# LeoIV/polyaxon

Measured on AMD Instinct MI355X. Metric: HPO trials/hour (whole node) + wall-clock-to-target, ResNet-50 Hyperband sweep, higher is better.
Workload: dtype bf16

## Files before the change

polyaxon_amd/csrc/bn_kernels.hip:

```cpp
#include <hip/hip_runtime.h>

#include "handoff.h"
#include <stdint.h>
#include <type_traits>

#define PLX_API extern "C" __attribute__((visibility("default")))

namespace {

constexpr int kBlock = 256;

struct alignas(16) bf16x8 {
  uint16_t v[8];
};

__device__ __forceinline__ float bf2f(uint16_t b) { return __uint_as_float(((uint32_t)b) << 16); }

__device__ __forceinline__ uint16_t f2bf(float f) {
  return __builtin_bit_cast(uint16_t, (__bf16)f);
}

__device__ __forceinline__ void load8(const bf16x8* p, float* f) {
  const bf16x8 v = *p;
#pragma unroll
// ... 81 lines not shown
                                                               float* __restrict__ out, int S) {
  constexpr int G = NT / 64;
  __shared__ float sh[NT];
  const int c = blockIdx.x * 64 + (threadIdx.x & 63);
  const int lane = threadIdx.x >> 6;
  const int s = blockIdx.y, which = blockIdx.z;
  const int b0 = s * kRowsPerSplit;
  const int b1 = b0 + kRowsPerSplit < nblk ? b0 + kRowsPerSplit : nblk;
  sh[threadIdx.x] = c < C ? l1_rows<NT>(part + (int64_t)which * nblk * C, b0, b1, C, c, lane) : 0.f;
  __syncthreads();
  if (lane == 0 && c < C) {
    float r = 0.f;
#pragma unroll
    for (int g = 0; g < G; ++g) r += sh[threadIdx.x + 64 * g];
    out[((int64_t)which * S + s) * C + c] = r;
  }
}

template <int NT = 256, bool ATOMIC = false>
__device__ __forceinline__ bool fin_sum2(const float* __restrict__ pa, const float* __restrict__ pb, int nblk, int C,
                                         double& A, double& B) {
  constexpr int G = NT / 64;
  __shared__ double sh[2][G][64];
  const int lc = threadIdx.x & 63, sp = threadIdx.x >> 6;
  const int c = blockIdx.x * 64 + lc;
  double a0 = 0.0, b0 = 0.0;
  if (c < C) {
    for (int b = sp; b < nblk; b += 8 * G) {
      float x[8], y[8];
#pragma unroll
      for (int u = 0; u < 8; ++u) {
        const int r = b + u * G;
        if (ATOMIC) {
          x[u] = r < nblk ? __hip_atomic_load(pa + (int64_t)r * C + c, __ATOMIC_RELAXED, __HIP_MEMORY_SCOPE_AGENT) : 0.f;
          y[u] = r < nblk ? __hip_atomic_load(pb + (int64_t)r * C + c, __ATOMIC_RELAXED, __HIP_MEMORY_SCOPE_AGENT) : 0.f;
        } else {
          x[u] = r < nblk ? pa[(int64_t)r * C + c] : 0.f;
          y[u] = r < nblk ? pb[(int64_t)r * C + c] : 0.f;
        }
      }
#pragma unroll
      for (int u = 0; u < 8; ++u) { a0 += x[u]; b0 += y[u]; }
    }
  }
  sh[0][sp][lc] = a0;
  sh[1][sp][lc] = b0;
  __syncthreads();
  if (sp != 0 || c >= C) return false;
  double sa = 0.0, sb = 0.0;
#pragma unroll
  for (int g = 0; g < G; ++g) { sa += sh[0][g][lc]; sb += sh[1][g][lc]; }
  A = sa;
  B = sb;
  return true;
}

struct FwdFin {
  const uint16_t* x_row0;
  int C;
  int64_t M;
  const float* gamma;
  const float* beta;
  float eps, momentum;
  float* running_mean;
  float* running_var;
  float* save_mean;
  float* save_invstd;
  float* scale;
  float* bias;
};

struct BwdFin {
  int C;
  int64_t M;
  const float* gamma;
  const float* mean;
  const float* invstd;
  float* dgamma;
  float* dbeta;
  float* coef;
  int accumulate;
};

template <int NT, bool ATOMIC = false>
__device__ __forceinline__ void fwd_finalize(const float* psum, const float* psq, int nblk, const FwdFin& f) {
  double S, Q;
  if (!fin_sum2<NT, ATOMIC>(psum, psq, nblk, f.C, S, Q)) return;
  const int c = blockIdx.x * 64 + (threadIdx.x & 63);
  const double m = S / (double)f.M;
  double var = Q / (double)f.M - m * m;
  if (var < 0.0) var = 0.0;
  const float mean = (f.x_row0 != nullptr ? bf2f(f.x_row0[c]) : 0.f) + (float)m;
  const float invstd = rsqrtf((float)var + f.eps);
  const float g = f.gamma[c];
  f.save_mean[c] = mean;
  f.save_invstd[c] = invstd;
  f.scale[c] = g * invstd;
  f.bias[c] = f.beta[c] - mean * g * invstd;
  if (f.running_mean != nullptr) {
    const float unbiased = f.M > 1 ? (float)(var * (double)f.M / (double)(f.M - 1)) : (float)var;
    f.running_mean[c] = (1.f - f.momentum) * f.running_mean[c] + f.momentum * mean;
    f.running_var[c] = (1.f - f.momentum) * f.running_var[c] + f.momentum * unbiased;
  }
}

template <int NT, bool ATOMIC = false>
__device__ __forceinline__ void bwd_finalize(const float* pdz, const float* pdzx, int nblk, const BwdFin& f) {
  double A, B;
  if (!fin_sum2<NT, ATOMIC>(pdz, pdzx, nblk, f.C, A, B)) return;
  const int C = f.C;
  const int c = blockIdx.x * 64 + (threadIdx.x & 63);
  const float db = (float)A, dg = (float)B;
  f.dbeta[c] = f.accumulate ? f.dbeta[c] + db : db;
  f.dgamma[c] = f.accumulate ? f.dgamma[c] + dg : dg;
  const float is = f.invstd[c], k1 = f.gamma[c] * is;
  const float k2 = db / (float)f.M, k3 = dg / (float)f.M;
  f.coef[c] = k1;
  f.coef[C + c] = -k1 * k3 * is;
  f.coef[2 * C + c] = -k1 * k2 + k1 * k3 * is * f.mean[c];
}

template <int NT>
__device__ __forceinline__ bool reduce_l2_last(const float* __restrict__ part, int nblk, int C, float* l2, int S,
                                               unsigned* cnt) {
  constexpr int G = NT / 64;
  __shared__ float sh[2][NT];
  __shared__ int s_last;
  const int c = blockIdx.x * 64 + (threadIdx.x & 63);
  const int lane = threadIdx.x >> 6;
  const int s = blockIdx.y;
  const int b0 = s * kRowsPerSplit;
  int b1 = b0 + kRowsPerSplit;
  if (b1 > nblk) b1 = nblk;
  float a0 = 0.f, a1 = 0.f;
  if (c < C) {
    a0 = l1_rows<NT>(part, b0, b1, C, c, lane);
    a1 = l1_rows<NT>(part + (int64_t)nblk * C, b0, b1, C, c, lane);
  }
  sh[0][threadIdx.x] = a0;
  sh[1][threadIdx.x] = a1;
  __syncthreads();
  if (lane == 0 && c < C) {
    const int t = threadIdx.x;
    float r0 = 0.f, r1 = 0.f;
#pragma unroll
    for (int g = 0; g < G; ++g) { r0 += sh[0][t + 64 * g]; r1 += sh[1][t + 64 * g]; }
    __hip_atomic_store(l2 + (int64_t)s * C + c, r0, __ATOMIC_RELAXED, __HIP_MEMORY_SCOPE_AGENT);
    __hip_atomic_store(l2 + ((int64_t)S + s) * C + c, r1, __ATOMIC_RELAXED, __HIP_MEMORY_SCOPE_AGENT);
  }
  asm volatile("s_waitcnt vmcnt(0)" ::: "memory");
  __syncthreads();
  if (threadIdx.x == 0) {
    plx_handoff_release();
    const unsigned old = __hip_atomic_fetch_add(cnt + blockIdx.x, 1u, __ATOMIC_RELAXED, __HIP_MEMORY_SCOPE_AGENT);
    const int last = old == (unsigned)(S - 1);
    if (last) plx_handoff_acquire();
    if (last) __hip_atomic_store(cnt + blockIdx.x, 0u, __ATOMIC_RELAXED, __HIP_MEMORY_SCOPE_AGENT);
    s_last = last;
  }
  __syncthreads();
  return s_last != 0;
}

constexpr int kFinNT = 1024;
template <int NT>
__global__ __launch_bounds__(NT) void bn_fwd_reduce_finalize_kernel(const float* __restrict__ part, int nblk, float* l2,
                                                                    int S, unsigned* cnt, FwdFin f) {
  if (!reduce_l2_last<NT>(part, nblk, f.C, l2, S, cnt)) return;
  fwd_finalize<NT, true>(l2, l2 + (int64_t)S * f.C, S, f);
}

template <int NT>
__global__ __launch_bounds__(NT) void bn_bwd_reduce_finalize_kernel(const float* __restrict__ part, int nblk, float* l2,
                                                                    int S, unsigned* cnt, BwdFin f) {
  if (!reduce_l2_last<NT>(part, nblk, f.C, l2, S, cnt)) return;
  bwd_finalize<NT, true>(l2, l2 + (int64_t)S * f.C, S, f);
}

template <int NT>
__global__ __launch_bounds__(NT) void bn_fwd_finalize_kernel(const float* __restrict__ psum, const float* __restrict__ psq, int nblk,
                                       const uint16_t* __restrict__ x_row0, int C, int64_t M,
                                       const float* __restrict__ gamma, const float* __restrict__ beta, float eps,
                                       float momentum, float* __restrict__ running_mean,
                                       float* __restrict__ running_var, float* __restrict__ save_mean,
                                       float* __restrict__ save_invstd, float* __restrict__ scale,
                                       float* __restrict__ bias) {
  double S, Q;
  if (!fin_sum2<NT>(psum, psq, nblk, C, S, Q)) return;
  const int c = blockIdx.x * 64 + (threadIdx.x & 63);
  const double m = S / (double)M;
  double var = Q / (double)M - m * m;
  if (var < 0.0) var = 0.0;
  const float mean = (x_row0 != nullptr ? bf2f(x_row0[c]) : 0.f) + (float)m;
  const float invstd = rsqrtf((float)var + eps);
  const float g = gamma[c];
  save_mean[c] = mean;
  save_invstd[c] = invstd;
  scale[c] = g * invstd;
  bias[c] = beta[c] - mean * g * invstd;
  if (running_mean != nullptr) {
    const float unbiased = M > 1 ? (float)(var * (double)M / (double)(M - 1)) : (float)var;
    running_mean[c] = (1.f - momentum) * running_mean[c] + momentum * mean;
    running_var[c] = (1.f - momentum) * running_var[c] + momentum * unbiased;
  }
}

template <bool RES, bool RELU>
__global__ __launch_bounds__(kBlock) void bn_apply_kernel(const bf16x8* __restrict__ x, const bf16x8* __restrict__ res,
                                                          bf16x8* __restrict__ y, const float* __restrict__ scale,
                                                          const float* __restrict__ bias, int64_t n_vec, int G,
                                                          uint8_t* __restrict__ mask, const float* __restrict__ rsb) {
  const int64_t stride = (int64_t)gridDim.x * blockDim.x;
  int64_t i = (int64_t)blockIdx.x * blockDim.x + threadIdx.x;
  if (i >= n_vec) return;
  const int cg = (int)(i % G);
  float a[8], b[8], ra[8], rb[8];
#pragma unroll
  for (int k = 0; k < 8; ++k) {
    a[k] = scale[cg * 8 + k];
    b[k] = bias[cg * 8 + k];
    ra[k] = 1.f;
    rb[k] = 0.f;
  }
  if (RES && rsb != nullptr) {
#pragma unroll
    for (int k = 0; k < 8; ++k) {
      ra[k] = rsb[cg * 8 + k];
      rb[k] = rsb[G * 8 + cg * 8 + k];
    }
  }
  for (; i < n_vec; i += stride) {
    const bf16x8 xv = x[i];
    bf16x8 rv;
    if constexpr (RES) rv = res[i];
    float v[8];
#pragma unroll
    for (int k = 0; k < 8; ++k) v[k] = fmaf(bf2f(xv.v[k]), a[k], b[k]);
    if constexpr (RES) {
#pragma unroll
      for (int k = 0; k < 8; ++k) v[k] += fmaf(bf2f(rv.v[k]), ra[k], rb[k]);
    }
    if constexpr (RELU) {
#pragma unroll
      for (int k = 0; k < 8; ++k) v[k] = fmaxf(v[k], 0.f);
    }
    store8(y + i, v);
    if (RELU && mask != nullptr) {
      uint32_t bits = 0;
#pragma unroll
      for (int k = 0; k < 8; ++k) bits |= (uint32_t)(v[k] > 0.f) << k;
      mask[i] = (uint8_t)bits;
    }
  }
}

template <bool RELU>
__global__ __launch_bounds__(kBlock) void bn_bwd_reduce_kernel(const bf16x8* __restrict__ x, const uint8_t* __restrict__ mask,
                                                               const bf16x8* __restrict__ dy, int64_t M, int G, int Gb,
                                                               int64_t rows_per_block, const float* __restrict__ mean,
// ... 138 lines not shown
  for (int k = 0; k < 8; ++k) {
    red[threadIdx.x * 16 + k] = ra[k];
    red[threadIdx.x * 16 + 8 + k] = rc[k];
  }
  __syncthreads();
  if ((int)threadIdx.x < G) {
    for (int j = 1; j < kBlock / G; ++j) {
      const float* o = red + (j * G + threadIdx.x) * 16;
#pragma unroll
      for (int k = 0; k < 8; ++k) {
        ra[k] += o[k];
        rc[k] += o[8 + k];
      }
    }
    float* pa = rb.part + (int64_t)blockIdx.x * C + cg * 8;
    float* pc = rb.part + ((int64_t)gridDim.x + blockIdx.x) * C + cg * 8;
#pragma unroll
    for (int k = 0; k < 8; ++k) {
      pa[k] = ra[k];
      pc[k] = rc[k];
    }
  }
  }
}

struct Plan {
  int G, Gb, gy, nblk, S;
  int64_t rows_per_block;
};

inline bool plan_for(int64_t M, int C, Plan* p) {
  if (M < 1 || C <= 0 || (C & 7)) return false;
  const int G = C / 8;
  if (G & (G - 1)) return false;
  p->G = G;
  p->Gb = G < kBlock ? G : kBlock;
  p->gy = G / p->Gb;
  const int R = kBlock / p->Gb;
  const int64_t cap = (2048 + p->gy - 1) / p->gy;
  int64_t want = (M + 16 * R - 1) / (16 * R);
  if (want > cap) want = cap;
  if (want < 1) want = 1;
  int64_t rpb = (M + want - 1) / want;
  rpb = (rpb + R - 1) / R * R;
  p->rows_per_block = rpb;
  p->nblk = (int)((M + rpb - 1) / rpb);
  p->S = (p->nblk + kRowsPerSplit - 1) / kRowsPerSplit;
  return true;
}

inline int apply_grid(int64_t n_vec, int G) {
  int64_t g = (n_vec + kBlock - 1) / kBlock;
  if (g > 4096) g = 4096;
  if (g < 1) g = 1;
  const int64_t mult = G > kBlock ? G / kBlock : 1;
  g = (g + mult - 1) / mult * mult;
  return (int)g;
}

inline void launch_dx(hipStream_t stream, int64_t n_vec, int G, const void* x, const uint8_t* mask, const void* dy,
                      void* dx, void* dres, const float* coef, int relu, const ResBn& rb) {
  const dim3 grid(apply_grid(n_vec, G));
  auto pick = [&](auto d) {
    constexpr bool DRES = decltype(d)::value;
    return rb.part == nullptr
               ? (relu ? bn_bwd_dx_kernel<false, true, false, DRES> : bn_bwd_dx_kernel<false, false, false, DRES>)
           : rb.mask != nullptr
               ? (relu ? bn_bwd_dx_kernel<true, true, true, DRES> : bn_bwd_dx_kernel<true, false, true, DRES>)
               : (relu ? bn_bwd_dx_kernel<true, true, false, DRES> : bn_bwd_dx_kernel<true, false, false, DRES>);
  };
  auto k = dres != nullptr ? pick(std::true_type{}) : pick(std::false_type{});
  hipLaunchKernelGGL(k, grid, dim3(kBlock), 0, stream, (const bf16x8*)x, mask, (const bf16x8*)dy, (bf16x8*)dx,
                     (bf16x8*)dres, coef, n_vec, G, relu, rb);
}

inline void launch_apply(hipStream_t stream, int64_t n_vec, int G, const void* x, const void* res, void* y,
                         const float* scale, const float* bias, int relu, uint8_t* mask, const float* rsb) {
  auto k = res != nullptr ? (relu ? bn_apply_kernel<true, true> : bn_apply_kernel<true, false>)
                          : (relu ? bn_apply_kernel<false, true> : bn_apply_kernel<false, false>);
  hipLaunchKernelGGL(k, dim3(apply_grid(n_vec, G)), dim3(kBlock), 0, stream, (const bf16x8*)x, (const bf16x8*)res,
                     (bf16x8*)y, scale, bias, n_vec, G, mask, rsb);
}

inline void reduce_finalize_fwd(hipStream_t stream, const float* part, int nblk, float* l2, unsigned* cnt,
                                const FwdFin& f) {
  const int C = f.C, S = (nblk + kRowsPerSplit - 1) / kRowsPerSplit;
  if (cnt != nullptr) {
    hipLaunchKernelGGL(bn_fwd_reduce_finalize_kernel<kFinNT>, dim3((C + 63) / 64, S), dim3(kFinNT), 0, stream, part, nblk, l2, S,
                       cnt, f);
    return;
  }
  hipLaunchKernelGGL(bn_partial_reduce_kernel<kFinNT>,
                     dim3((C + 63) / 64, S, 2), dim3(kFinNT), 0, stream, part, nblk, C, l2, S);
  hipLaunchKernelGGL(bn_fwd_finalize_kernel<kFinNT>, dim3((C + 63) / 64),
                     dim3(kFinNT), 0, stream, l2, l2 + (int64_t)S * C, S,
                     f.x_row0, C, f.M, f.gamma, f.beta, f.eps, f.momentum, f.running_mean, f.running_var, f.save_mean,
                     f.save_invstd, f.scale, f.bias);
}

inline void reduce_finalize_bwd(hipStream_t stream, const float* part, int nblk, float* l2, unsigned* cnt,
                                const BwdFin& f) {
  const int C = f.C, S = (nblk + kRowsPerSplit - 1) / kRowsPerSplit;
  if (cnt != nullptr) {
    hipLaunchKernelGGL(bn_bwd_reduce_finalize_kernel<kFinNT>, dim3((C + 63) / 64, S), dim3(kFinNT), 0, stream, part, nblk, l2, S,
                       cnt, f);
    return;
  }
  hipLaunchKernelGGL(bn_partial_reduce_kernel<kFinNT>,
                     dim3((C + 63) / 64, S, 2), dim3(kFinNT), 0, stream, part, nblk, C, l2, S);
  hipLaunchKernelGGL(bn_bwd_finalize_kernel<kFinNT>, dim3((C + 63) / 64),
                     dim3(kFinNT), 0, stream, l2, l2 + (int64_t)S * C, S, C,
                     f.M, f.gamma, f.mean, f.invstd, f.dgamma, f.dbeta, f.coef, f.accumulate);
}

struct alignas(8) u8x8 {
  uint8_t v[8];
};

__global__ __launch_bounds__(256) void stem_apply_pool_kernel(const bf16x8* __restrict__ x,
                                                              const float* __restrict__ sb, bf16x8* __restrict__ y,
                                                              u8x8* __restrict__ idx, int N, int H, int W, int G,
                                                              int OH, int OW) {
  const unsigned j = blockIdx.x * 256u + threadIdx.x;
  if (j >= (unsigned)(OW * G)) return;
  const unsigned g = j % (unsigned)G, ow = j / (unsigned)G;
  const int C = G * 8;
  float a[8], b[8];
#pragma unroll
  for (int k = 0; k < 8; ++k) {
    a[k] = sb[g * 8 + k];
    b[k] = sb[C + g * 8 + k];
  }
  for (int row = blockIdx.y; row < N * OH; row += gridDim.y) {
    const int n = row / OH, oh = row - n * OH;
    float best[8];
    uint8_t arg[8];
#pragma unroll
    for (int k = 0; k < 8; ++k) {
      best[k] = -INFINITY;
      arg[k] = 255;
    }
    uint4 q[9];
    bool ok[9];
#pragma unroll
    for (int kh = 0; kh < 3; ++kh) {
      const int ih = oh * 2 - 1 + kh;
      const int ihc = ih < 0 ? 0 : (ih >= H ? H - 1 : ih);
#pragma unroll
      for (int kw = 0; kw < 3; ++kw) {
        const int iw = (int)ow * 2 - 1 + kw;
        const int iwc = iw < 0 ? 0 : (iw >= W ? W - 1 : iw);
        ok[kh * 3 + kw] = ih >= 0 && ih < H && iw >= 0 && iw < W;
        q[kh * 3 + kw] = *(const uint4*)(x + ((size_t)(n * H + ihc) * W + iwc) * G + g);
      }
    }
#pragma unroll
    for (int t9 = 0; t9 < 9; ++t9) {
      const uint32_t qw[4] = {q[t9].x, q[t9].y, q[t9].z, q[t9].w};
#pragma unroll
      for (int k = 0; k < 8; ++k) {
        const float xk = __uint_as_float((k & 1) ? (qw[k >> 1] & 0xffff0000u) : (qw[k >> 1] << 16));
        const float f = (float)(__bf16)fmaxf(fmaf(xk, a[k], b[k]), 0.f);
        if (ok[t9] && (f > best[k] || arg[k] == 255)) {
          best[k] = f;
          arg[k] = (uint8_t)t9;
        }
      }
    }
    bf16x8 o;
    u8x8 m;
#pragma unroll
    for (int k = 0; k < 8; ++k) {
      o.v[k] = f2bf(best[k]);
      m.v[k] = arg[k];
    }
    const size_t t = (size_t)row * OW * G + j;
    y[t] = o;
    idx[t] = m;
  }
}

__device__ __forceinline__ int stem_cover(int i, int O, int* o, int* k) {
  int n = 0;
  if (i & 1) {
    if ((i + 1) >> 1 < O) { o[n] = (i + 1) >> 1; k[n++] = 0; }
// ... 292 lines not shown
    for (int h = 0; h < 2; ++h) {
      float cst[NA][4];
#pragma unroll
      for (int arr = 0; arr < NA; ++arr) {
        const float4 v = thin_lds[(arr * 2 + h) * G + g];
        cst[arr][0] = v.x, cst[arr][1] = v.y, cst[arr][2] = v.z, cst[arr][3] = v.w;
      }
      thin_pin4(amw[0][h], amw[1][h], amw[2][h], amw[3][h]);
#pragma unroll
      for (int kp = 0; kp < 2; ++kp) {
        const int w = h * 2 + kp;
        thin_pin4(dw[0][w], dw[1][w], dw[2][w], dw[3][w]);
        thin_pin4(xw[0][w], xw[1][w], xw[2][w], xw[3][w]);
#pragma unroll
        for (int k2 = 0; k2 < 2; ++k2) {
          const int kk = kp * 2 + k2, k = h * 4 + kk;
#pragma unroll
          for (int e = 0; e < 4; ++e) {
            const int di = e >> 1, dj = e & 1;
            float acc = 0.f;
#pragma unroll
            for (int p = 0; p < 2; ++p)
#pragma unroll
              for (int q = 0; q < 2; ++q) {
                const int kh = di + 1 - 2 * p, kw = dj + 1 - 2 * q;
                if (kh < 0 || kw < 0) continue;
                const int w4 = p * 2 + q;
                const uint32_t ab = amw[w4][h] >> (8 * kk) & 0xffu;
                const float dv = __uint_as_float(k2 ? (dw[w4][w] & 0xffff0000u) : (dw[w4][w] << 16));
                acc += ab == (uint32_t)(kh * 3 + kw) ? dv : 0.f;
              }
            const float xf = __uint_as_float(k2 ? (xw[e][w] & 0xffff0000u) : (xw[e][w] << 16));
            const float dz = (pv[e] && fmaf(xf, cst[0][kk], cst[1][kk]) > 0.f) ? (float)(__bf16)acc : 0.f;
            if constexpr (DX) {
              const uint32_t ob = f2bf(fmaf(cst[2][kk], dz, fmaf(cst[3][kk], xf, cst[NA - 1][kk])));
              ow4[e][w] = k2 ? (ow4[e][w] | (ob << 16)) : ob;
            } else {
              s1[k] += dz;
              s2[k] = fmaf(dz, (xf - cst[2][kk]) * cst[3][kk], s2[k]);
            }
          }
        }
        if constexpr (DX) thin_pin4(ow4[0][w], ow4[1][w], ow4[2][w], ow4[3][w]);
        thin_sched_fence();
      }
    }
    if constexpr (DX) {
#pragma unroll
      for (int e = 0; e < 4; ++e)
        if (pv[e])
          *(uint4*)(dx + ((size_t)(n * H + 2 * qa + (e >> 1)) * W + 2 * qb + (e & 1)) * G + g) =
              make_uint4(ow4[e][0], ow4[e][1], ow4[e][2], ow4[e][3]);
    }
  }
  if constexpr (!DX) {
    __shared__ float red[256 * 17];
#pragma unroll
    for (int k = 0; k < 8; ++k) {
      red[threadIdx.x * 17 + k] = s1[k];
      red[threadIdx.x * 17 + 8 + k] = s2[k];
    }
    __syncthreads();
    const int nb = gridDim.x * gridDim.y, blk = blockIdx.y * gridDim.x + blockIdx.x;
    for (int e = threadIdx.x; e < G * 16; e += 256) {
      const int gg = e % G, v = e / G;
      float sum = 0.f;
      for (int r = gg; r < 256; r += G) sum += red[r * 17 + v];
      const int c = gg * 8 + (v & 7);
      part[((int64_t)(v < 8 ? 0 : nb) + blk) * C + c] = sum;
    }
  }
}

constexpr int g_stem_bwd_cap = 4096;

inline dim3 stem_bwd_grid(int N, int H, int W, int G, bool dx) {
  const int rows = N * ((H + 1) / 2), cap = dx ? 65535 : g_stem_bwd_cap;
  return dim3((((W + 1) / 2) * G + 255) / 256, rows < cap ? rows : cap);
}

}

PLX_API void plx_bn_set_thin(int on) { g_bn_thin = on != 0; }

PLX_API int64_t plx_bn_workspace(int64_t M, int C) {
  Plan p;
  if (!plan_for(M, C, &p)) return -1;
  return 2 * (int64_t)(p.nblk + p.S) * C;
}

PLX_API int64_t plx_bn_l2_workspace(int nblk, int C) {
  return 2 * (int64_t)((nblk + kRowsPerSplit - 1) / kRowsPerSplit) * C;
}

PLX_API int plx_bn_dx_blocks(int64_t M, int C) {
  Plan p;
  if (!plan_for(M, C, &p)) return -1;
  return apply_grid(M * p.G, p.G);
}

struct BnForwardArgs {
  const void *x, *res;
  void* y;
  int64_t M;
  int C, relu;
  const float *gamma, *beta;
  float eps, momentum;
  float *running_mean, *running_var;
  float *save_mean, *save_invstd, *scale_bias , *workspace;
  const float* ext_part;
  int ext_nblk;
  uint8_t* mask;
  const float* res_sb;
  unsigned* counters;
};

struct BnBackwardArgs {
  const void* x;
  const uint8_t* mask;
  const void* dy;
  void* dx;
  void* dres;
  int64_t M;
  int C, relu;
  const float *gamma, *save_mean, *save_invstd;
  float *dgamma, *dbeta, *coef , *workspace;
  const float* ext_part;
  int ext_nblk, accumulate;
  ResBn resbn;
  unsigned* counters;
  int no_dres;
};

PLX_API int plx_bn_args_size(int backward) {
  return (int)(backward ? sizeof(BnBackwardArgs) : sizeof(BnForwardArgs));
}

PLX_API int plx_bn_forward(const BnForwardArgs* a, hipStream_t stream) {
  Plan p;
  const int C = a->C;
  if (!plan_for(a->M, C, &p) || (a->ext_part != nullptr && a->ext_nblk < 1)) return 1;
  const bool own = a->ext_part == nullptr;
  const int nblk = own ? p.nblk : a->ext_nblk;
  float* l2 = own ? a->workspace + 2 * (int64_t)nblk * C : a->workspace;
  if (own)
    hipLaunchKernelGGL(bn_stats_kernel, dim3(p.nblk, p.gy), dim3(kBlock), 0, stream, (const bf16x8*)a->x, a->M, p.G,
                       p.Gb, p.rows_per_block, a->workspace, a->workspace + (int64_t)nblk * C);
  reduce_finalize_fwd(stream, own ? a->workspace : a->ext_part, nblk, l2, a->counters,
                      FwdFin{own ? (const uint16_t*)a->x : nullptr, C, a->M, a->gamma, a->beta, a->eps, a->momentum, a->running_mean,
                             a->running_var, a->save_mean, a->save_invstd, a->scale_bias, a->scale_bias + C});
  if (a->y != nullptr)
    launch_apply(stream, a->M * p.G, p.G, a->x, a->res, a->y, a->scale_bias, a->scale_bias + C, a->relu,
                 a->relu ? a->mask : nullptr, a->res_sb);
  return (int)hipGetLastError();
}

PLX_API int plx_bn_backward(const BnBackwardArgs* a, hipStream_t stream) {
  Plan p;
  const int C = a->C, relu = a->relu;
  const ResBn& rb = a->resbn;
  const bool has_rb = rb.x != nullptr || rb.mask != nullptr || rb.mean != nullptr || rb.invstd != nullptr ||
                      rb.part != nullptr;
  if (!plan_for(a->M, C, &p) || (a->ext_part != nullptr && a->ext_nblk < 1)) return 1;
  if (relu && a->mask == nullptr && (a->ext_part == nullptr || a->dx != nullptr)) return 1;
  if (has_rb && (rb.part == nullptr || rb.x == nullptr || rb.mean == nullptr || rb.invstd == nullptr)) return 1;
  if (has_rb && (a->dres == nullptr) != (a->no_dres != 0)) return 1;
// ... 105 lines not shown
```

polyaxon_amd/ops/_native.py:

```python
from __future__ import annotations

import ctypes
import hashlib
import os
import shutil
import subprocess
import threading
from pathlib import Path
from typing import Dict, Iterable, List, Optional

PKG_DIR = Path(__file__).resolve().parent.parent
CSRC = PKG_DIR / "csrc"
OUT = PKG_DIR / "_native"
ARCH = os.environ.get("PLX_OFFLOAD_ARCH", "gfx950")
ROCM = Path(os.environ.get("ROCM_PATH", "/opt/rocm"))

LIBRARIES: Dict[str, dict] = {
    "plx_train": {"sources": ["train_kernels.hip"], "kind": "hip", "link": []},
    "plx_polytune": {"sources": ["polytune_kernels.hip"], "kind": "hip", "link": []},
    "plx_bn": {"sources": ["bn_kernels.hip"], "kind": "hip", "link": []},
    "plx_procmon": {"sources": ["procmon.cpp"], "kind": "cpp", "link": ["-lpthread"]},
    "plx_gp": {"sources": ["gp_kernels.hip", "gp_chol.hip"], "kind": "hip", "link": []},
    "plx_rms": {"sources": ["rmsnorm.hip"], "kind": "hip", "link": []},
    "plx_conv": {"sources": ["conv_gemm.hip"], "kind": "hip", "link": []},
# ... 65 lines not shown
    return out


def _stale(name: str) -> bool:
    spec = LIBRARIES[name]
    stamp = lib_path(name).with_suffix(".so.sha")
    if not stamp.exists():
        return False
    try:
        digest = _digest([CSRC / s for s in spec["sources"]], _flags(spec["kind"]) + spec["link"])
    except OSError:
        return False
    return stamp.read_text().strip() != digest


def build_all(force: bool = False, verbose: bool = False) -> List[Path]:
    return [build(n, force=force, verbose=verbose) for n in LIBRARIES]


def available(name: str) -> bool:
    return lib_path(name).exists()


_SIZES: Dict[tuple, int] = {}


_COUNTERS: Dict[tuple, object] = {}


def capturing() -> bool:
    import torch

    return torch.cuda.is_available() and torch.cuda.is_current_stream_capturing()


def cached(cache: dict, key, make, ok=None):
    v = cache.get(key)
    if v is not None and (ok is None or ok(v)):
        return v
    v = make()
    if not capturing():
        cache[key] = v
    return v


def counters(device, key: str, n: int = 4096):
    import torch

    return cached(_COUNTERS, (str(device), key), lambda: torch.zeros(n, dtype=torch.int32, device=device))


def current_stream() -> int:
    import torch

    return torch._C._cuda_getCurrentRawStream(torch._C._cuda_getDevice())


def size(libname: str, fn: str, *args: int) -> int:
    key = (fn,) + args
    v = _SIZES.get(key)
    if v is None:
        v = _SIZES[key] = int(getattr(lib(libname), fn)(*args))
    return v


def lib(name: str) -> ctypes.CDLL:
    with _lock:
        if name in _loaded:
            return _loaded[name]
        path = lib_path(name)
        if not path.exists() or os.environ.get("PLX_NATIVE_REBUILD") == "1" or _stale(name):
            build(name, force=os.environ.get("PLX_NATIVE_REBUILD") == "1")
        handle = ctypes.CDLL(str(path), mode=ctypes.RTLD_GLOBAL)
        _declare(name, handle)
        if name == "plx_bn":
            for backward, image in enumerate((BnForwardArgs, BnBackwardArgs)):
                if handle.plx_bn_args_size(backward) != ctypes.sizeof(image):
                    raise RuntimeError(f"{image.__name__} layout mismatch: HIP {handle.plx_bn_args_size(backward)} vs "
                                       f"ctypes {ctypes.sizeof(image)}")
        if name == "plx_conv" and os.environ.get("PLX_WGRAD_ATOMIC"):
            handle.plx_set_tn_atomic(int(os.environ["PLX_WGRAD_ATOMIC"]))
        if name == "plx_bn" and os.environ.get("PLX_BN_THIN"):
            handle.plx_bn_set_thin(int(os.environ["PLX_BN_THIN"]))
        if name == "plx_gemm" and os.environ.get("PLX_GEMM_WAVES"):
            handle.plx_gemm256_set_waves(int(os.environ["PLX_GEMM_WAVES"]))
        _loaded[name] = handle
        return handle


_P = ctypes.c_void_p
_I = ctypes.c_int
_L = ctypes.c_int64
_U64 = ctypes.c_uint64
_F = ctypes.c_float
_D = ctypes.c_double

SIGNATURES: Dict[str, Dict[str, list]] = {
    "plx_train": {
        "plx_sgd_flat": [_P, _P, _P, _L, _L, _P, _P, _P],
        "plx_adamw_flat": [_P, _P, _P, _P, _L, _L, _P, _P, _P],
        "plx_adamw_mixed": [_P, _P, _P, _P, _P, _L, _I, _P, _P, _P],
        "plx_sgd_flat_clip": [_P, _P, _P, _L, _L, _P, _P, _P, _P],
        "plx_adamw_flat_clip": [_P, _P, _P, _P, _L, _L, _P, _P, _P, _P],
        "plx_adamw_mixed_clip": [_P, _P, _P, _P, _P, _L, _I, _P, _P, _P, _P],
        "plx_gradnorm_blocks": [_L],
        "plx_gradnorm_partials": [_P, _I, _L, _P, _P],
        "plx_gradnorm_finalize": [_P, _I, _P, _P, _P],
        "plx_lr_schedule": [_P, _P, _P, _P],
        "plx_cast_lp": [_P, _P, _L, _P],
        "plx_init_flat": [_P, _P, _P, _P, _I, _P, _P, _U64, _P],
        "plx_zero_flat": [_P, _L, _P],
        "plx_record_metric": [_P, _I, _P, _P, _I, _P],
        "plx_commit_metric": [_P, _P, _I, _I, _P, _I, _P],
        "plx_synth_images": [_P, _P, _I, _I, _I, _P, _I, _I, _F, _U64, _P, _P],
        "plx_set_adamw_grid_cap": [_I],
        "plx_set_adamw_wide": [_I],
    },
    "plx_bn": {
        "plx_bn_set_thin": [_I],
        "plx_bn_workspace": [_L, _I],
        "plx_bn_args_size": [_I],
        "plx_bn_forward": [_P, _P],
        "plx_bn_apply": [_P, _P, _P, _L, _I, _P, _I, _P],
        "plx_bn_apply_res_relu": [_P, _P, _P, _L, _I, _P, _P, _P, _P],
        "plx_bn_l2_workspace": [_I, _I],
        "plx_bn_backward": [_P, _P],
        "plx_bn_dx_blocks": [_L, _I],
        "plx_stem_bn_pool_forward": [_P, _P, _P, _I, _I, _I, _I, _P, _P, _F, _F, _P, _P, _P, _P, _P, _P, _P, _I, _P,
                                     _P],
        "plx_stem_bn_pool_bwd_workspace": [_I, _I, _I, _I],
        "plx_stem_bn_pool_backward": [_P, _P, _P, _P, _I, _I, _I, _I, _P, _P, _P, _P, _P, _P, _P, _P, _I, _P, _P],
    },
    "plx_procmon": {
        "plx_pm_create": [],
        "plx_pm_destroy": [_P],
        "plx_pm_spawn": [_P, _P, _P, ctypes.c_char_p, ctypes.c_char_p, ctypes.POINTER(_I)],
        "plx_pm_wait": [_P, _I, ctypes.POINTER(_I), ctypes.POINTER(_I)],
        "plx_pm_wake": [_P],
        "plx_pm_signal": [_P, _I, _I, _I],
        "plx_pm_count": [_P],
    },
    "plx_gp": {
        "plx_gp_kmat": [_P, _P, _I, _I, _I, _P, _I, _I, _F, _F, _F, _I, _F, _P, _P, _D, _I, _P],
        "plx_gp_chol": [_P, _I, _I, _P, _P],
        "plx_gp_kmat_batch_f64": [_P, _I, _I, _P, _I, _P, _I, _L, _I, _D, _D, _D, _P, _P, _D, _I, _P],
        "plx_gp_matern_table": [_D, _D, _D, _I, _P, _P, _P],
        "plx_gp_chol_aug_f64": [_P, _I, _I, _I, _L, _I, _P, _P, _P],
        "plx_gp_chol_scratch_doubles": [],
        "plx_gp_lml_f64": [_P, _I, _I, _L, _I, _P, _P, _P],
        "plx_gp_acq_rows": [_P, _I, _I, _P, _F, _I, _F, _F, _F, _P, _P, _P, _P],
        "plx_gp_predict_acq": [_P, _I, _P, _I, _I, _P, _I, _P, _I, _F, _F, _F, _F, _I, _F, _F, _F, _P, _P, _P, _P,
                               _P, _P, _P, _D, _I, _P],
        "plx_gp_ascent": [_P, _P, _I, _P, _P, _P, _I, _I, _P, _P, _I, _F, _F, _F, _F, _I, _F, _F, _F, _I, _P, _P, _D, _I,
                          _P],
    },
    "plx_conv": {
        "plx_gemm_nt": [_P, _P, _P, _I, _I, _I, _I, _I, _I, _P, _P, _I, _P, _P, _P],
        "plx_gemm_nt_bndx": [_P, _P, _P, _P, _P, _P, _P, _I, _I, _I, _I, _I, _P, _I, _P, _P, _P],
        "plx_gemm_nt_bndx_wgrad": [_P, _P, _P, _P, _P, _P, _P, _I, _I, _I, _I, _I, _P, _I, _P, _P, _P, _P, _I, _I, _P],
        "plx_gemm_nt_bnapply": [_P, _P, _P, _P, _P, _P, _P, _P, _I, _I, _I, _I, _I, _P, _P],
        "plx_gemm_nt_rows_per_block": [_I],
        "plx_gemm_nt_plan": [_I, _I, _I, _I],
        "plx_gemm_tn_workspace": [_I, _I, _I, _I],
        "plx_set_tn_v2": [_I, _I],
        "plx_set_tn2_stem": [_I],
        "plx_set_tn2_c64": [_I],
        "plx_set_tn_atomic": [_I],
        "plx_get_tn_atomic": [],
        "plx_tn_plan_slices": [_I, _I, _I, _I, _I],
        "plx_gemm_tn": [_P, _P, _P, _P, _I, _I, _I, _I, _I, _I, _I, _I, _P],
        "plx_weight_prep": [_P, _P, _P, _I, _I, _P],
        "plx_weight_prepk": [_P, _L, _L, _L, _L, _P, _P, _I, _I, _I, _P],
        "plx_weight_prep_all": [_P, _P, _P, _P, _I, _I, _P],
        "plx_stem_pack_input": [_P, _P, _I, _I, _I, _P],
        "plx_stem_pack_weight": [_P, _L, _L, _L, _L, _P, _I, _P],
        "plx_stem_conv_fwd": [_P, _P, _P, _I, _I, _I, _P, _P],
        "plx_stem_conv_wgrad_workspace": [_I, _I, _I, _I],
        "plx_stem_conv_wgrad": [_P, _P, _P, _L, _L, _L, _L, _P, _I, _I, _I, _I, _I, _P],
        "plx_conv_fwd": [_P, _P, _P, _I, _I, _I, _I, _I, _I, _I, _P, _P],
        "plx_conv_dgrad": [_P, _P, _P, _I, _I, _I, _I, _I, _I, _I, _P, _P, _P],
        "plx_conv_dgrad_blocks": [_I, _I, _I, _I, _I, _I, _I],
        "plx_conv_wgrad_workspace": [_I, _I, _I, _I, _I, _I, _I, _I],
        "plx_conv_wgrad": [_P, _P, _P, _P, _I, _I, _I, _I, _I, _I, _I, _I, _I, _P],
    },
    "plx_lm": {
        "plx_qkv_rope_fwd": [_P, _P, _P, _P, _P, _P, _L, _I, _I, _I, _I, _I, _P],
        "plx_qkv_rope_bwd": [_P, _P, _P, _P, _P, _P, _L, _I, _I, _I, _I, _I, _P],
        "plx_swiglu_fwd": [_P, _P, _L, _I, _P],
        "plx_swiglu_bwd": [_P, _P, _P, _L, _I, _P],
        "plx_xent_fwd": [_P, _P, _P, _P, _I, _I, _I, _P],
        "plx_xent_bwd": [_P, _P, _P, _P, _P, _I, _I, _I, _P],
        "plx_xent_cls_fwd": [_P, _P, _P, _P, _I, _I, _P],
        "plx_xent_cls_bwd": [_P, _P, _P, _P, _P, _I, _I, _F, _P],
        "plx_xent_hp_fwd": [_P, _P, _P, _P, _P, _P, _I, _I, _I, _I, _P],
        "plx_xent_hp_bwd": [_P, _P, _P, _P, _P, _P, _I, _I, _I, _I, _P],
        "plx_xent_cls_hp_fwd": [_P, _P, _P, _P, _P, _P, _I, _I, _I, _P],
        "plx_xent_cls_hp_bwd": [_P, _P, _P, _P, _P, _P, _I, _I, _I, _F, _P],
        "plx_colsum_splits": [_L, _I],
        "plx_colsum": [_P, _L, _I, _P, _P, _P, _I, _P],
        "plx_gelu_bwd_colsum": [_P, _P, _P, _L, _I, _P, _P, _P, _I, _P],
    },
    "plx_gemm": {
# ... 113 lines not shown
```

Measured before the change: 13290.

## Add single-kernel BN stat finalize replacing ticket-based split reduction

Adds a single-launch finalize path for BN forward and backward. When the partial-row count is small, one 1024-thread block per 64 channels reduces all partial sums through shared memory, which removes the multi-block atomic ticket handoff and the L2 scratch round-trip. Per-channel parameters (gamma, beta, running stats, and so on) are now prefetched with bounds-checked buffer loads issued alongside the partial loads, so their latency overlaps the reduction. The ticket path also switches to buffer loads. The trade-off is fewer blocks in flight on the reduction, which lowers parallelism for large channel counts, plus more code paths to keep correct.

Measured after the change: 13460, median of 6. 1.01x the previous value.

```diff
diff --git a/polyaxon_amd/csrc/bn_kernels.hip b/polyaxon_amd/csrc/bn_kernels.hip
--- a/polyaxon_amd/csrc/bn_kernels.hip
+++ b/polyaxon_amd/csrc/bn_kernels.hip
@@ -187,42 +187,104 @@
   int accumulate;
 };
 
-template <int NT, bool ATOMIC = false>
-__device__ __forceinline__ void fwd_finalize(const float* psum, const float* psq, int nblk, const FwdFin& f) {
-  double S, Q;
-  if (!fin_sum2<NT, ATOMIC>(psum, psq, nblk, f.C, S, Q)) return;
-  const int c = blockIdx.x * 64 + (threadIdx.x & 63);
+struct FwdPar {
+  float gamma, beta, rmean, rvar, x0;
+};
+
+struct BwdPar {
+  float gamma, mean, invstd, dgamma, dbeta;
+};
+
+__device__ __forceinline__ __amdgpu_buffer_rsrc_t buf_rsrc(const void* p, int bytes) {
+  return __builtin_amdgcn_make_buffer_rsrc(const_cast<void*>(p), 0, bytes, 0x00020000);
+}
+
+__device__ __forceinline__ float par_load(const float* p, int C, int c, bool on) {
+  const int bytes = p != nullptr ? C * (int)sizeof(float) : 0;
+  return __uint_as_float(__builtin_amdgcn_raw_buffer_load_b32(buf_rsrc(p, bytes), on ? c * (int)sizeof(float) : bytes, 0, 0));
+}
+
+__device__ __forceinline__ FwdPar fwd_params(const FwdFin& f, int c, bool on) {
+  FwdPar p;
+  p.gamma = par_load(f.gamma, f.C, c, on);
+  p.beta = par_load(f.beta, f.C, c, on);
+  p.rmean = par_load(f.running_mean, f.C, c, on);
+  p.rvar = par_load(f.running_mean != nullptr ? f.running_var : nullptr, f.C, c, on);
+  const int xbytes = f.x_row0 != nullptr ? 2 * f.C : 0;
+  p.x0 = bf2f((uint16_t)__builtin_amdgcn_raw_buffer_load_b16(buf_rsrc(f.x_row0, xbytes), on ? 2 * c : xbytes, 0, 0));
+  return p;
+}
+
+__device__ __forceinline__ BwdPar bwd_params(const BwdFin& f, int c, bool on) {
+  BwdPar p;
+  p.gamma = par_load(f.gamma, f.C, c, on);
+  p.mean = par_load(f.mean, f.C, c, on);
+  p.invstd = par_load(f.invstd, f.C, c, on);
+  p.dgamma = par_load(f.dgamma, f.C, c, on);
+  p.dbeta = par_load(f.dbeta, f.C, c, on);
+  return p;
+}
+
+__device__ __forceinline__ void fwd_finish(const FwdFin& f, int c, double S, double Q, const FwdPar& p) {
   const double m = S / (double)f.M;
   double var = Q / (double)f.M - m * m;
   if (var < 0.0) var = 0.0;
-  const float mean = (f.x_row0 != nullptr ? bf2f(f.x_row0[c]) : 0.f) + (float)m;
+  const float mean = p.x0 + (float)m;
   const float invstd = rsqrtf((float)var + f.eps);
-  const float g = f.gamma[c];
+  const float g = p.gamma;
   f.save_mean[c] = mean;
   f.save_invstd[c] = invstd;
   f.scale[c] = g * invstd;
-  f.bias[c] = f.beta[c] - mean * g * invstd;
+  f.bias[c] = p.beta - mean * g * invstd;
   if (f.running_mean != nullptr) {
     const float unbiased = f.M > 1 ? (float)(var * (double)f.M / (double)(f.M - 1)) : (float)var;
-    f.running_mean[c] = (1.f - f.momentum) * f.running_mean[c] + f.momentum * mean;
-    f.running_var[c] = (1.f - f.momentum) * f.running_var[c] + f.momentum * unbiased;
-  }
-}
-
-template <int NT, bool ATOMIC = false>
-__device__ __forceinline__ void bwd_finalize(const float* pdz, const float* pdzx, int nblk, const BwdFin& f) {
-  double A, B;
-  if (!fin_sum2<NT, ATOMIC>(pdz, pdzx, nblk, f.C, A, B)) return;
+    f.running_mean[c] = (1.f - f.momentum) * p.rmean + f.momentum * mean;
+    f.running_var[c] = (1.f - f.momentum) * p.rvar + f.momentum * unbiased;
+  }
+}
+
+__device__ __forceinline__ void bwd_finish(const BwdFin& f, int c, double A, double B, const BwdPar& p) {
   const int C = f.C;
-  const int c = blockIdx.x * 64 + (threadIdx.x & 63);
   const float db = (float)A, dg = (float)B;
-  f.dbeta[c] = f.accumulate ? f.dbeta[c] + db : db;
-  f.dgamma[c] = f.accumulate ? f.dgamma[c] + dg : dg;
-  const float is = f.invstd[c], k1 = f.gamma[c] * is;
+  f.dbeta[c] = f.accumulate ? p.dbeta + db : db;
+  f.dgamma[c] = f.accumulate ? p.dgamma + dg : dg;
+  const float is = p.invstd, k1 = p.gamma * is;
   const float k2 = db / (float)f.M, k3 = dg / (float)f.M;
   f.coef[c] = k1;
   f.coef[C + c] = -k1 * k3 * is;
-  f.coef[2 * C + c] = -k1 * k2 + k1 * k3 * is * f.mean[c];
+  f.coef[2 * C + c] = -k1 * k2 + k1 * k3 * is * p.mean;
+}
+
+template <int NT, bool ATOMIC = false>
+__device__ __forceinline__ void fwd_finalize(const float* psum, const float* psq, int nblk, const FwdFin& f,
+                                             const FwdPar& p) {
+  double S, Q;
+  if (!fin_sum2<NT, ATOMIC>(psum, psq, nblk, f.C, S, Q)) return;
+  fwd_finish(f, blockIdx.x * 64 + (threadIdx.x & 63), S, Q, p);
+}
+
+template <int NT, bool ATOMIC = false>
+__device__ __forceinline__ void bwd_finalize(const float* pdz, const float* pdzx, int nblk, const BwdFin& f,
+                                             const BwdPar& p) {
+  double A, B;
+  if (!fin_sum2<NT, ATOMIC>(pdz, pdzx, nblk, f.C, A, B)) return;
+  bwd_finish(f, blockIdx.x * 64 + (threadIdx.x & 63), A, B, p);
+}
+
+template <int NT>
+__device__ __forceinline__ float l1_rows_buf(const float* __restrict__ src, int b0, int b1, int C, int c, int lane) {
+  constexpr int G = NT / 64, U = kRowsPerSplit / G;
+  const int bytes = (b1 - b0) * C * (int)sizeof(float);
+  const __amdgpu_buffer_rsrc_t r = buf_rsrc(src + (int64_t)b0 * C, bytes);
+  float x[U];
+#pragma unroll
+  for (int u = 0; u < U; ++u)
+    x[u] = __uint_as_float(__builtin_amdgcn_raw_buffer_load_b32(
+        r, c < C ? ((lane + u * G) * C + c) * (int)sizeof(float) : bytes, 0, 0));
+  float a = 0.f;
+#pragma unroll
+  for (int u = 0; u < U; ++u) a += x[u];
+  return a;
 }
 
 template <int NT>
@@ -237,11 +299,8 @@
   const int b0 = s * kRowsPerSplit;
   int b1 = b0 + kRowsPerSplit;
   if (b1 > nblk) b1 = nblk;
-  float a0 = 0.f, a1 = 0.f;
-  if (c < C) {
-    a0 = l1_rows<NT>(part, b0, b1, C, c, lane);
-    a1 = l1_rows<NT>(part + (int64_t)nblk * C, b0, b1, C, c, lane);
-  }
+  const float a0 = l1_rows_buf<NT>(part, b0, b1, C, c, lane);
+  const float a1 = l1_rows_buf<NT>(part + (int64_t)nblk * C, b0, b1, C, c, lane);
   sh[0][threadIdx.x] = a0;
   sh[1][threadIdx.x] = a1;
   __syncthreads();
@@ -271,15 +330,102 @@
 template <int NT>
 __global__ __launch_bounds__(NT) void bn_fwd_reduce_finalize_kernel(const float* __restrict__ part, int nblk, float* l2,
                                                                     int S, unsigned* cnt, FwdFin f) {
+  const int c = blockIdx.x * 64 + (threadIdx.x & 63);
+  const FwdPar p = fwd_params(f, c, threadIdx.x < 64 && c < f.C);
   if (!reduce_l2_last<NT>(part, nblk, f.C, l2, S, cnt)) return;
-  fwd_finalize<NT, true>(l2, l2 + (int64_t)S * f.C, S, f);
+  fwd_finalize<NT, true>(l2, l2 + (int64_t)S * f.C, S, f, p);
 }
 
 template <int NT>
 __global__ __launch_bounds__(NT) void bn_bwd_reduce_finalize_kernel(const float* __restrict__ part, int nblk, float* l2,
                                                                     int S, unsigned* cnt, BwdFin f) {
+  const int c = blockIdx.x * 64 + (threadIdx.x & 63);
+  const BwdPar p = bwd_params(f, c, threadIdx.x < 64 && c < f.C);
   if (!reduce_l2_last<NT>(part, nblk, f.C, l2, S, cnt)) return;
-  bwd_finalize<NT, true>(l2, l2 + (int64_t)S * f.C, S, f);
+  bwd_finalize<NT, true>(l2, l2 + (int64_t)S * f.C, S, f, p);
+}
+
+constexpr int kFinSingleSplits = 8;
+constexpr int kFinSingleMax = kFinSingleSplits * kRowsPerSplit;
+
+template <int CW, int SM, typename F>
+__device__ __forceinline__ bool single_sum2(const float* __restrict__ part, int nblk, int C, double& A, double& B,
+                                            F&& load_params) {
+  constexpr int NT = kFinNT;
+  constexpr int NSUB = 64 / CW;
+  constexpr int KS = SM / NSUB;
+  constexpr int RS = CW == 64 && SM > 4 ? 4 : SM;
+  static_assert(NT / CW == 16 * NSUB && SM % NSUB == 0 && SM % RS == 0 && 2 * RS * CW <= NT && SM <= 16, "mapping");
+  __shared__ float sh[2][RS][16][CW];
+  __shared__ float rs[2][SM][CW];
+  const int t = threadIdx.x;
+  const int lc = t % CW, j = t / CW, g = j & 15, sub = j >> 4;
+  const int c = blockIdx.x * CW + lc;
+  const int bytes = 2 * nblk * C * (int)sizeof(float);
+  const __amdgpu_buffer_rsrc_t src = buf_rsrc(part, bytes);
+  float x[2][KS][4];
+#pragma unroll
+  for (int w = 0; w < 2; ++w)
+#pragma unroll
+    for (int k = 0; k < KS; ++k)
+#pragma unroll
+      for (int u = 0; u < 4; ++u) {
+        const int b = (sub + NSUB * k) * kRowsPerSplit + g + 16 * u;
+        const int off = ((w * nblk + b) * C + c) * (int)sizeof(float);
+        x[w][k][u] = __uint_as_float(__builtin_amdgcn_raw_buffer_load_b32(src, b < nblk && c < C ? off : bytes, 0, 0));
+      }
+  load_params();
+  __builtin_amdgcn_sched_barrier(0);
+#pragma unroll
+  for (int r0 = 0; r0 < SM; r0 += RS) {
+    if (r0 != 0) __syncthreads();
+#pragma unroll
+    for (int w = 0; w < 2; ++w)
+#pragma unroll
+      for (int k = 0; k < KS; ++k) {
+        float a = 0.f;
+#pragma unroll
+        for (int u = 0; u < 4; ++u) a += x[w][k][u];
+        const int s = sub + NSUB * k;
+        if (s >= r0 && s < r0 + RS) sh[w][s - r0][g][lc] = a;
+      }
+    __syncthreads();
+    if (t < 2 * RS * CW) {
+      const int w = t / (RS * CW), sl = t / CW % RS;
+      float r = 0.f;
+#pragma unroll
+      for (int gg = 0; gg < 16; ++gg) r += sh[w][sl][gg][lc];
+      rs[w][r0 + sl][lc] = r;
+    }
+  }
+  __syncthreads();
+  if (t >= CW || c >= C) return false;
+  double sa = 0.0, sb = 0.0;
+#pragma unroll
+  for (int s = 0; s < SM; ++s) { sa += (double)rs[0][s][t]; sb += (double)rs[1][s][t]; }
+  A = sa;
+  B = sb;
+  return true;
+}
+
+template <int CW, int SM>
+__global__ __launch_bounds__(kFinNT) void bn_fwd_finalize_single_kernel(const float* __restrict__ part, int nblk,
+                                                                        FwdFin f) {
+  const int c = blockIdx.x * CW + threadIdx.x % CW;
+  FwdPar p;
+  double S, Q;
+  if (!single_sum2<CW, SM>(part, nblk, f.C, S, Q, [&] { p = fwd_params(f, c, threadIdx.x < CW && c < f.C); })) return;
+  fwd_finish(f, c, S, Q, p);
+}
+
+template <int CW, int SM>
+__global__ __launch_bounds__(kFinNT) void bn_bwd_finalize_single_kernel(const float* __restrict__ part, int nblk,
+                                                                        BwdFin f) {
+  const int c = blockIdx.x * CW + threadIdx.x % CW;
+  BwdPar p;
+  double A, B;
+  if (!single_sum2<CW, SM>(part, nblk, f.C, A, B, [&] { p = bwd_params(f, c, threadIdx.x < CW && c < f.C); })) return;
+  bwd_finish(f, c, A, B, p);
 }
 
 template <int NT>
@@ -584,9 +730,23 @@
                      (bf16x8*)y, scale, bias, n_vec, G, mask, rsb);
 }
 
+int g_bn_fin_single = 1;
+
+enum { kFinTwoLaunch = 0, kFinTicket = 1, kFinSingle = 2 };
+
+inline int fin_path(int nblk, int C, bool counters) {
+  if (!counters) return kFinTwoLaunch;
+  return g_bn_fin_single && nblk <= kFinSingleMax && (int64_t)nblk * C < (1 << 28) ? kFinSingle : kFinTicket;
+}
+
 inline void reduce_finalize_fwd(hipStream_t stream, const float* part, int nblk, float* l2, unsigned* cnt,
                                 const FwdFin& f) {
   const int C = f.C, S = (nblk + kRowsPerSplit - 1) / kRowsPerSplit;
+  if (fin_path(nblk, C, cnt != nullptr) == kFinSingle) {
+    auto k = S <= 2 ? bn_fwd_finalize_single_kernel<64, 2> : bn_fwd_finalize_single_kernel<64, kFinSingleSplits>;
+    hipLaunchKernelGGL(k, dim3((C + 63) / 64), dim3(kFinNT), 0, stream, part, nblk, f);
+    return;
+  }
   if (cnt != nullptr) {
     hipLaunchKernelGGL(bn_fwd_reduce_finalize_kernel<kFinNT>, dim3((C + 63) / 64, S), dim3(kFinNT), 0, stream, part, nblk, l2, S,
                        cnt, f);
@@ -603,6 +763,11 @@
 inline void reduce_finalize_bwd(hipStream_t stream, const float* part, int nblk, float* l2, unsigned* cnt,
                                 const BwdFin& f) {
   const int C = f.C, S = (nblk + kRowsPerSplit - 1) / kRowsPerSplit;
+  if (fin_path(nblk, C, cnt != nullptr) == kFinSingle) {
+    auto k = S <= 2 ? bn_bwd_finalize_single_kernel<64, 2> : bn_bwd_finalize_single_kernel<64, kFinSingleSplits>;
+    hipLaunchKernelGGL(k, dim3((C + 63) / 64), dim3(kFinNT), 0, stream, part, nblk, f);
+    return;
+  }
   if (cnt != nullptr) {
     hipLaunchKernelGGL(bn_bwd_reduce_finalize_kernel<kFinNT>, dim3((C + 63) / 64, S), dim3(kFinNT), 0, stream, part, nblk, l2, S,
                        cnt, f);
@@ -1061,6 +1226,13 @@
 }
 
 PLX_API void plx_bn_set_thin(int on) { g_bn_thin = on != 0; }
+
+PLX_API void plx_bn_set_fin_single(int on) { g_bn_fin_single = on != 0; }
+
+PLX_API int plx_bn_fin_path(int nblk, int C) {
+  if (nblk < 1 || C < 8 || C % 8 || ((C / 8) & (C / 8 - 1))) return -1;
+  return fin_path(nblk, C, true);
+}
 
 PLX_API int64_t plx_bn_workspace(int64_t M, int C) {
   Plan p;
diff --git a/polyaxon_amd/ops/_native.py b/polyaxon_amd/ops/_native.py
--- a/polyaxon_amd/ops/_native.py
+++ b/polyaxon_amd/ops/_native.py
@@ -171,6 +171,8 @@
             handle.plx_set_tn_atomic(int(os.environ["PLX_WGRAD_ATOMIC"]))
         if name == "plx_bn" and os.environ.get("PLX_BN_THIN"):
             handle.plx_bn_set_thin(int(os.environ["PLX_BN_THIN"]))
+        if name == "plx_bn" and os.environ.get("PLX_BN_FIN_SINGLE"):
+            handle.plx_bn_set_fin_single(int(os.environ["PLX_BN_FIN_SINGLE"]))
         if name == "plx_gemm" and os.environ.get("PLX_GEMM_WAVES"):
             handle.plx_gemm256_set_waves(int(os.environ["PLX_GEMM_WAVES"]))
         _loaded[name] = handle
@@ -207,6 +209,8 @@
     },
     "plx_bn": {
         "plx_bn_set_thin": [_I],
+        "plx_bn_set_fin_single": [_I],
+        "plx_bn_fin_path": [_I, _I],
         "plx_bn_workspace": [_L, _I],
         "plx_bn_args_size": [_I],
         "plx_bn_forward": [_P, _P],
```
